# Connor-Guo/torcheval

Hardware: AMD Instinct MI355X
Metric: metric-updates/sec (whole node) MulticlassAccuracy bs=8192 at 1/2/4/8 MI355X (higher is better)
Workload: dtype fp32; 1 GPU; model=MulticlassAccuracy, global_batch=8192, num_classes=1000, batch_per_gpu=8192, average=micro, parallelism=dp1

## Files before the change

csrc/bindings/counts.cpp:

```cpp
#include <ATen/ATen.h>
#include <torch/csrc/utils/pybind.h>
#include <torch/library.h>

#include "tea_kernels.h"
#include "tea_torch.h"

namespace {

using namespace tea_torch;

void cls_counts(const Tensor& input, const Tensor& target, int64_t k, int64_t num_classes,
                const optional<Tensor>& micro_correct, const optional<Tensor>& micro_total,
                const optional<Tensor>& cls_correct, const optional<Tensor>& cls_label,
                const optional<Tensor>& cls_pred, const optional<Tensor>& confusion,
                const optional<Tensor>& err, int64_t max_blocks,
                const optional<Tensor>& micro_incorrect, const optional<Tensor>& micro_total2,
                const optional<Tensor>& cls_fp) {
  check_gpu(input, "input");
  check_gpu(target, "target");
  TORCH_CHECK(target.dim() == 1, "cls_counts: target must be 1-D");
  TORCH_CHECK(input.dim() == 1 || input.dim() == 2, "cls_counts: input must be 1-D or 2-D");
  TORCH_CHECK(input.size(0) == target.size(0), "cls_counts: first dims differ");
  TORCH_CHECK(target.is_contiguous(), "cls_counts: target must be contiguous");
  DeviceGuard guard(input.device());
  tea::ClsCountsArgs a;
  Tensor in = input;
  if (input.dim() == 2) {
    if (in.stride(1) != 1) in = in.contiguous();
    a.c = in.size(1);
    a.row_stride = in.stride(0);
    TORCH_CHECK(a.c < (int64_t(1) << 31), "cls_counts: too many classes");
    TORCH_CHECK(k >= 1 && k <= a.c || a.c == 0, "cls_counts: k out of range");
    if (num_classes <= 0) num_classes = a.c;
    TORCH_CHECK(num_classes == a.c, "cls_counts: num_classes must match input.size(1)");
  } else {
    if (!in.is_contiguous()) in = in.contiguous();
    TORCH_CHECK(k == 1, "cls_counts: k > 1 needs 2-D scores");
  }
  const int64_t C = num_classes;
  a.input = in.data_ptr();
  a.in_dt = dt_of(in);
  a.n = in.size(0);
  a.target = target.data_ptr();
  a.tg_dt = dt_of(target);
  a.k = static_cast<int>(k);
  a.num_classes = C;
  a.micro_correct = f32_out(micro_correct, input, 1, "micro_correct");
  a.micro_total = f32_out(micro_total, input, 1, "micro_total");
  a.cls_correct = f32_out(cls_correct, input, C, "cls_correct");
  a.cls_label = f32_out(cls_label, input, C, "cls_label");
  a.cls_pred = f32_out(cls_pred, input, C, "cls_pred");
  a.confusion = f32_out(confusion, input, C * C, "confusion");
  a.micro_incorrect = f32_out(micro_incorrect, input, 1, "micro_incorrect");
  a.micro_total2 = f32_out(micro_total2, input, 1, "micro_total2");
  a.cls_fp = f32_out(cls_fp, input, C, "cls_fp");
  TORCH_CHECK(!(k > 1 && (a.cls_pred || a.confusion || a.cls_fp)),
              "cls_counts: predictions are undefined for k > 1");
  TORCH_CHECK((a.cls_correct || a.cls_label || a.cls_pred || a.confusion || a.cls_fp) == false ||
                  C > 0,
              "cls_counts: num_classes required for histograms");
  if ((a.err = err_ptr(err, input, "cls_counts")) != nullptr) {
    if (err->numel() >= 3) a.err_max = a.err + 1;
    a.check_target = 1;
  }
  a.max_blocks = static_cast<int>(max_blocks);
  const hipStream_t stream = stream_for(input);
  if (a.micro_correct || a.micro_incorrect) a.fold_ws = fold_workspace(input, stream);
  const int rc = tea::launch_cls_counts(a, stream);
  TORCH_CHECK(rc != -1, "cls_counts: unsupported input dtype ", input.scalar_type());
  check_launch(rc, "cls_counts");
}

bool micro_accuracy_update(const Tensor& input, const Tensor& target, const Tensor& correct,
                           const Tensor& total, int64_t num_classes, const optional<Tensor>& pend) {
  if (!input.is_cuda() || input.dim() != 2 || target.dim() != 1) return false;
  const int64_t n = input.size(0), c = input.size(1);
  if (target.size(0) != n || c <= 0 || c >= (int64_t(1) << 31) || input.stride(1) != 1) return false;
  if (num_classes > 0 && c != num_classes) return false;
  const auto st = input.scalar_type();
  if (st != at::kFloat && st != at::kBFloat16 && st != at::kHalf) return false;
  switch (target.scalar_type()) {
    case at::kLong: case at::kInt: case at::kShort: case at::kChar: case at::kByte: case at::kBool:
      break;
    default: return false;
  }
  if (!target.is_contiguous()) return false;
  const auto dev = input.device();
  if (target.device() != dev || correct.device() != dev || total.device() != dev) return false;
  if (correct.scalar_type() != at::kFloat || total.scalar_type() != at::kFloat ||
      correct.numel() != 1 || total.numel() != 1)
    return false;
  DeviceGuard guard(dev);
  tea::ClsCountsArgs a;
  a.input = input.data_ptr();
  a.in_dt = dt_of(input);
  a.n = n;
  a.c = c;
  a.row_stride = input.stride(0);
  a.target = target.data_ptr();
  a.tg_dt = dt_of(target);
  a.k = 1;
  a.num_classes = c;
  a.micro_correct = correct.data_ptr<float>();
  a.micro_total = total.data_ptr<float>();
  const hipStream_t stream = stream_for(input);
  if (pend.has_value()) {
    if (pend->scalar_type() != at::kLong || pend->numel() < tea::kPendCells * tea::kPendStride ||
        pend->device() != dev || !pend->is_contiguous())
      return false;
    a.pend = reinterpret_cast<unsigned long long*>(pend->data_ptr<int64_t>());
  } else {
    a.fold_ws = fold_workspace(input, stream);
  }
  check_launch(tea::launch_cls_counts(a, stream), "micro_accuracy_update");
  return true;
}

void micro_accuracy_finish(const Tensor& pend, const Tensor& correct, const Tensor& total,
                           const optional<Tensor>& out) {
  check_gpu(pend, "pend");
  TORCH_CHECK(pend.scalar_type() == at::kLong && pend.is_contiguous() &&
                  pend.numel() >= tea::kPendCells * tea::kPendStride,
              "micro_accuracy_finish: pend must be int64 [>= 512]");
  TORCH_CHECK(correct.scalar_type() == at::kFloat && total.scalar_type() == at::kFloat && correct.numel() == 1 &&
                  total.numel() == 1 && correct.device() == pend.device() && total.device() == pend.device(),
              "micro_accuracy_finish: float32 scalar states on the pending cells' device");
  float* o = nullptr;
  if (out.has_value()) {
    TORCH_CHECK(out->scalar_type() == at::kFloat && out->numel() == 1 && out->device() == pend.device(),
                "micro_accuracy_finish: out must be a float32 scalar");
    o = out->data_ptr<float>();
  }
  DeviceGuard guard(pend.device());
  check_launch(tea::launch_micro_finish(reinterpret_cast<unsigned long long*>(pend.data_ptr<int64_t>()),
                                        correct.data_ptr<float>(), total.data_ptr<float>(), o, stream_for(pend)),
               "micro_accuracy_finish");
}

Tensor rank_scores(const Tensor& input, const Tensor& target, int64_t mode, int64_t k,
                   const optional<Tensor>& err) {
  check_gpu(input, "input");
  check_gpu(target, "target");
  TORCH_CHECK(input.dim() == 2 && target.dim() == 1 && input.size(0) == target.size(0),
              "rank_scores: input [n, c] and target [n] expected");
  TORCH_CHECK(mode == 0 || mode == 1, "rank_scores: mode must be 0 (hit) or 1 (reciprocal)");
  TORCH_CHECK(input.size(1) < (int64_t(1) << 31), "rank_scores: too many columns");
  DeviceGuard guard(input.device());
  Tensor in = input.stride(1) == 1 ? input : input.contiguous();
  Tensor tg = target.contiguous();
  tea::RankArgs a;
  a.input = in.data_ptr();
  a.in_dt = dt_of(in);
  a.n = in.size(0);
  a.c = in.size(1);
  a.row_stride = in.stride(0);
  a.target = tg.data_ptr();
  a.tg_dt = dt_of(tg);
  a.mode = static_cast<int>(mode);
  a.k = static_cast<int>(k);
  Tensor out = at::empty({a.n}, input.options().dtype(at::kFloat));
  a.out = out.data_ptr<float>();
  a.err = err_ptr(err, input, "rank_scores");
  const int rc = tea::launch_rank_scores(a, stream_for(input));
  TORCH_CHECK(rc != -1, "rank_scores: unsupported input dtype ", input.scalar_type());
  check_launch(rc, "rank_scores");
  return out;
}

void binary_counts(const Tensor& input, const Tensor& target, const optional<Tensor>& weight,
                   double threshold, const optional<Tensor>& tp, const optional<Tensor>& fp,
                   const optional<Tensor>& tn, const optional<Tensor>& fn,
                   const optional<Tensor>& total, int64_t strict, int64_t max_blocks,
                   const optional<Tensor>& tp2, const optional<Tensor>& fp2,
                   const optional<Tensor>& tn2, const optional<Tensor>& fn2) {
  check_gpu(input, "input");
  check_gpu(target, "target");
  TORCH_CHECK(input.numel() == target.numel(), "binary_counts: size mismatch");
  DeviceGuard guard(input.device());
  Tensor in = input.contiguous();
  Tensor tg = target.contiguous();
  Tensor w;
  tea::BinaryCountsArgs a;
  if (weight.has_value()) {
    w = weight->contiguous();
    TORCH_CHECK(w.numel() == in.numel(), "binary_counts: weight size mismatch");
    a.weight = w.data_ptr();
    a.w_dt = dt_of(w);
  }
  a.input = in.data_ptr();
  a.in_dt = dt_of(in);
  a.target = tg.data_ptr();
  a.tg_dt = dt_of(tg);
  a.n = in.numel();
  a.threshold = threshold_as(in, threshold);
  a.threshold64 = threshold;
  a.strict_binary = static_cast<int>(strict);
  a.out[0] = f32_out(tp, input, 1, "tp");
  a.out[1] = f32_out(fp, input, 1, "fp");
  a.out[2] = f32_out(tn, input, 1, "tn");
  a.out[3] = f32_out(fn, input, 1, "fn");
  a.total = f32_out(total, input, 1, "total");
  a.out2[0] = f32_out(tp2, input, 1, "tp2");
  a.out2[1] = f32_out(fp2, input, 1, "fp2");
  a.out2[2] = f32_out(tn2, input, 1, "tn2");
  a.out2[3] = f32_out(fn2, input, 1, "fn2");
  a.max_blocks = static_cast<int>(max_blocks);
// ... 134 lines not shown
  check_launch(rc, "sample_binned_auroc");
}

void binned_finalize(const Tensor& tp, const Tensor& fp, const optional<Tensor>& fn,
                     const optional<Tensor>& out_auroc, const optional<Tensor>& out_auprc,
                     const optional<Tensor>& out_prec, const optional<Tensor>& out_rec) {
  check_gpu(tp, "tp");
  TORCH_CHECK(tp.dim() == 2 && tp.scalar_type() == at::kFloat && fp.sizes() == tp.sizes() &&
                  fp.strides() == tp.strides() && fp.scalar_type() == at::kFloat,
              "binned_finalize: tp/fp must be float32 [T, rows] with equal strides");
  DeviceGuard guard(tp.device());
  tea::BinnedFinalizeArgs a;
  a.tp = tp.data_ptr<float>();
  a.fp = fp.data_ptr<float>();
  a.k_stride = tp.stride(0);
  a.r_stride = tp.stride(1);
  a.T = static_cast<int>(tp.size(0));
  a.rows = tp.size(1);
  if (out_auprc.has_value()) {
    TORCH_CHECK(fn.has_value() && fn->sizes() == tp.sizes() && fn->strides() == tp.strides() &&
                    fn->scalar_type() == at::kFloat, "binned_finalize: AUPRC needs fn like tp");
    TORCH_CHECK(out_auprc->scalar_type() == at::kFloat && out_auprc->is_contiguous() &&
                    out_auprc->numel() == a.rows, "binned_finalize: out_auprc float32 [rows]");
    a.fn = fn->data_ptr<float>();
    a.out_auprc = out_auprc->data_ptr<float>();
  }
  if (out_auroc.has_value()) {
    TORCH_CHECK(out_auroc->scalar_type() == at::kDouble && out_auroc->is_contiguous() &&
                    out_auroc->numel() == a.rows, "binned_finalize: out_auroc float64 [rows]");
    a.out_auroc = out_auroc->data_ptr<double>();
  }
  if (out_prec.has_value() || out_rec.has_value()) {
    TORCH_CHECK(out_prec.has_value() && out_rec.has_value() && fn.has_value() &&
                    fn->sizes() == tp.sizes() && fn->strides() == tp.strides() &&
                    fn->scalar_type() == at::kFloat,
                "binned_finalize: a curve needs fn like tp and both out_prec / out_rec");
    for (const Tensor* o : {&*out_prec, &*out_rec})
      TORCH_CHECK(o->scalar_type() == at::kFloat && o->is_contiguous() &&
                      o->numel() == a.rows * (a.T + 1) && o->device() == tp.device(),
                  "binned_finalize: curve outputs must be contiguous float32 [rows, T + 1]");
    a.fn = fn->data_ptr<float>();
    a.out_prec = out_prec->data_ptr<float>();
    a.out_rec = out_rec->data_ptr<float>();
  }
  check_launch(tea::launch_binned_finalize(a, stream_for(tp)), "binned_finalize");
}

void op_cls_counts(const Tensor& input, const Tensor& target, int64_t k, int64_t num_classes,
                   const optional<Tensor>& micro_correct, const optional<Tensor>& micro_total,
                   const optional<Tensor>& cls_correct, const optional<Tensor>& cls_label,
                   const optional<Tensor>& cls_pred, const optional<Tensor>& confusion,
                   const optional<Tensor>& err) {
  cls_counts(input, target, k, num_classes, micro_correct, micro_total, cls_correct, cls_label, cls_pred,
             confusion, err, 0, c10::nullopt, c10::nullopt, c10::nullopt);
}
void op_micro_accuracy(const Tensor& input, const Tensor& target, const Tensor& correct, const Tensor& total) {
  TORCH_CHECK(micro_accuracy_update(input, target, correct, total, 0, c10::nullopt),
              "micro_accuracy: unsupported input (needs [N, C] f32/bf16/f16 scores with unit column stride, "
              "[N] integer targets and float32 scalar states on one ROCm device)");
}
void op_binary_counts(const Tensor& input, const Tensor& target, const optional<Tensor>& weight, double threshold,
                      const optional<Tensor>& tp, const optional<Tensor>& fp, const optional<Tensor>& tn,
                      const optional<Tensor>& fn, const optional<Tensor>& total, int64_t strict) {
  binary_counts(input, target, weight, threshold, tp, fp, tn, fn, total, strict, 0, c10::nullopt, c10::nullopt,
                c10::nullopt, c10::nullopt);
}
void op_binned_counts(const Tensor& input, const Tensor& target, const Tensor& thr, int64_t mode, const Tensor& tp,
                      const Tensor& fp, const Tensor& fn, int64_t uniform) {
  binned_counts(input, target, thr, mode, tp, fp, fn, uniform);
}

}

void tea_bind_counts(py::module_& m) {
  m.def("rank_scores", &rank_scores, "K10 rank-of-target scores (hit rate / reciprocal rank)", py::arg("input"),
        py::arg("target"), py::arg("mode"), py::arg("k"), py::arg("err") = py::none());
  m.def("micro_accuracy_update", &micro_accuracy_update,
        "K1 micro accuracy (k=1) accumulated into float32 scalar states; false = not handled", py::arg("input"),
        py::arg("target"), py::arg("correct"), py::arg("total"), py::arg("num_classes") = 0,
        py::arg("pend") = py::none());
  m.def("micro_accuracy_finish", &micro_accuracy_finish,
        "fold the micro kernel's pending cells into correct (and write correct / total to out)", py::arg("pend"),
        py::arg("correct"), py::arg("total"), py::arg("out") = py::none());
  m.def("cls_counts", &cls_counts, "K1 fused classification counts", py::arg("input"), py::arg("target"), py::arg("k"),
        py::arg("num_classes"), py::arg("micro_correct"), py::arg("micro_total"), py::arg("cls_correct"),
        py::arg("cls_label"), py::arg("cls_pred"), py::arg("confusion"), py::arg("err"), py::arg("max_blocks") = 0,
        py::arg("micro_incorrect") = py::none(), py::arg("micro_total2") = py::none(), py::arg("cls_fp") = py::none());
  m.def("binary_counts", &binary_counts, "K1b thresholded binary counts", py::arg("input"), py::arg("target"),
        py::arg("weight"), py::arg("threshold"), py::arg("tp"), py::arg("fp"), py::arg("tn"), py::arg("fn"),
        py::arg("total"), py::arg("strict") = 0, py::arg("max_blocks") = 0, py::arg("tp2") = py::none(),
        py::arg("fp2") = py::none(), py::arg("tn2") = py::none(), py::arg("fn2") = py::none());
  m.def("multilabel_counts", &multilabel_counts, "K2 multilabel accuracy counts", py::arg("input"), py::arg("target"),
        py::arg("threshold"), py::arg("k"), py::arg("criteria"), py::arg("num_correct"),
        py::arg("num_total") = py::none(), py::arg("total") = 0.0);
  m.def("binned_counts", &binned_counts, "K4 binned TP/FP/FN per (threshold, class)", py::arg("input"),
        py::arg("target"), py::arg("thr"), py::arg("mode"), py::arg("tp"), py::arg("fp"), py::arg("fn"),
        py::arg("uniform") = 0);
  m.def("sample_binned_auroc", &sample_binned_auroc,
        "K4b per-sample multiclass binned AUROC (the reference default), labels checked into err", py::arg("input"),
        py::arg("target"), py::arg("thr"), py::arg("out"), py::arg("err"));
  m.def("binned_finalize", &binned_finalize, "binned AUROC / AUPRC / PR-curve points from counts", py::arg("tp"),
        py::arg("fp"), py::arg("fn") = py::none(), py::arg("out_auroc") = py::none(), py::arg("out_auprc") = py::none(),
        py::arg("out_prec") = py::none(), py::arg("out_rec") = py::none());
}

TORCH_LIBRARY_FRAGMENT(torcheval_amd, m) {
  m.def("micro_accuracy(Tensor input, Tensor target, Tensor(a!) correct, Tensor(b!) total) -> ()");
  m.def("cls_counts(Tensor input, Tensor target, int k, int num_classes, Tensor(a!)? micro_correct, "
        "Tensor(b!)? micro_total, Tensor(c!)? cls_correct, Tensor(d!)? cls_label, Tensor(e!)? cls_pred, "
        "Tensor(f!)? confusion, Tensor(g!)? err) -> ()");
  m.def("binary_counts(Tensor input, Tensor target, Tensor? weight, float threshold, Tensor(a!)? tp, "
        "Tensor(b!)? fp, Tensor(c!)? tn, Tensor(d!)? fn, Tensor(e!)? total, int strict) -> ()");
  m.def("multilabel_counts(Tensor input, Tensor target, float threshold, int k, int criteria, "
        "Tensor(a!) num_correct, Tensor(b!)? num_total, float total) -> ()");
  m.def("rank_scores(Tensor input, Tensor target, int score_mode, int k, Tensor(a!)? err) -> Tensor");
  m.def("binned_counts(Tensor input, Tensor target, Tensor thr, int target_mode, Tensor(a!) tp, Tensor(b!) fp, "
        "Tensor(c!) fn, int uniform) -> ()");
  m.def("binned_finalize(Tensor tp, Tensor fp, Tensor? fn, Tensor(a!)? out_auroc, Tensor(b!)? out_auprc, "
        "Tensor(c!)? out_prec, Tensor(d!)? out_rec) -> ()");
}

TORCH_LIBRARY_IMPL(torcheval_amd, CUDA, m) {
  m.impl("micro_accuracy", &op_micro_accuracy);
  m.impl("cls_counts", &op_cls_counts);
  m.impl("binary_counts", &op_binary_counts);
  m.impl("multilabel_counts", &multilabel_counts);
  m.impl("rank_scores", &rank_scores);
  m.impl("binned_counts", &op_binned_counts);
  m.impl("binned_finalize", &binned_finalize);
}

TORCH_LIBRARY_IMPL(torcheval_amd, Meta, m) {
  m.impl("micro_accuracy", &MetaNoop<&op_micro_accuracy>::call);
  m.impl("cls_counts", &MetaNoop<&op_cls_counts>::call);
  m.impl("binary_counts", &MetaNoop<&op_binary_counts>::call);
  m.impl("multilabel_counts", &MetaNoop<&multilabel_counts>::call);
  m.impl("rank_scores", [](const Tensor& input, const Tensor&, int64_t, int64_t, const optional<Tensor>&) {
    return at::empty({input.size(0)}, input.options().dtype(at::kFloat));
  });
  m.impl("binned_counts", &MetaNoop<&op_binned_counts>::call);
  m.impl("binned_finalize", &MetaNoop<&binned_finalize>::call);
}
```

csrc/include/tea_kernels.h:

```cpp
#pragma once

#include <hip/hip_runtime_api.h>
#include <stdint.h>

#include "tea_types.h"

namespace tea {

struct ClsCountsArgs {
  const void* input = nullptr;
  DType in_dt = DType::f32;
  int64_t n = 0;
  int64_t c = 0;
  int64_t row_stride = 0;
  const void* target = nullptr;
  DType tg_dt = DType::i64;
  int k = 1;
  int64_t num_classes = 0;
  float* micro_correct = nullptr;
  float* micro_incorrect = nullptr;
  float* micro_total = nullptr;
  float* micro_total2 = nullptr;
  float* cls_correct = nullptr;
  float* cls_label = nullptr;
  float* cls_pred = nullptr;
  float* cls_fp = nullptr;
  float* confusion = nullptr;
  int* err = nullptr;
  int* err_max = nullptr;
  int check_target = 0;
  unsigned long long* fold_ws = nullptr;
  unsigned long long* pend = nullptr;
  int max_blocks = 0;
};
int launch_cls_counts(const ClsCountsArgs& a, hipStream_t stream);
constexpr int kPendCells = 64;
constexpr int kPendStride = 8;
int launch_micro_finish(unsigned long long* pend, float* correct, const float* total, float* out, hipStream_t stream);

struct BinaryCountsArgs {
  const void* input = nullptr;
  DType in_dt = DType::f32;
  const void* target = nullptr;
  DType tg_dt = DType::f32;
  const void* weight = nullptr;
  DType w_dt = DType::f32;
  int64_t n = 0;
  float threshold = 0.5f;
  double threshold64 = 0.5;
  int strict_binary = 0;
  float* out[4] = {nullptr, nullptr, nullptr, nullptr};
  float* out2[4] = {nullptr, nullptr, nullptr, nullptr};
  float* total = nullptr;
  int max_blocks = 0;
};
int launch_binary_counts(const BinaryCountsArgs& a, hipStream_t stream);

struct RankArgs {
  const void* input = nullptr;
  DType in_dt = DType::f32;
  int64_t n = 0;
  int64_t c = 0;
  int64_t row_stride = 0;
  const void* target = nullptr;
  DType tg_dt = DType::i64;
  int mode = 0;
  int k = 0;
  float* out = nullptr;
  int* err = nullptr;
};
int launch_rank_scores(const RankArgs& a, hipStream_t stream);

}

namespace tea {

struct AucScanArgs {
  int payload_kind = 0;
  const void* sorted = nullptr;
  DType key_dt = DType::f32;
  int64_t key_stride = 0;
  const int64_t* order = nullptr;
  const int32_t* order32 = nullptr;
  int64_t order_stride = 0;
  const void* target = nullptr;
  DType tg_dt = DType::f32;
  int64_t target_stride = 0;
  const void* weight = nullptr;
  DType w_dt = DType::f32;
  int64_t weight_stride = 0;
  int class_mode = 0;
  int64_t rows = 0;
  int64_t n = 0;
  double* out_auroc = nullptr;
  double* out_auprc = nullptr;
  const uint32_t* sort_fault = nullptr;
  const double* init = nullptr;
  double* out_raw = nullptr;
  void* ab = nullptr;
  void* tsum = nullptr;
  void* tstart = nullptr;
  void* tarea = nullptr;
  void* totals = nullptr;
  int32_t* tcnt = nullptr;
  int32_t* cstart = nullptr;
  int64_t* sizes = nullptr;
  const int64_t* row_off = nullptr;
  float* out_prec = nullptr;
  float* out_rec = nullptr;
  void* out_thr = nullptr;
  float min_precision = 0.f;
  float* s_rec = nullptr;
  void* s_thr = nullptr;
  int32_t* gstar = nullptr;
  int32_t* glo = nullptr;
  float* out_max_recall = nullptr;
  void* out_best_thr = nullptr;
};
int64_t auc_scan_workspace_bytes(int64_t rows, int64_t n);
int launch_auc_scan(AucScanArgs a, void* workspace, hipStream_t stream);
// ... 418 lines not shown
```

csrc/kernels/classification.hip:

```cpp
#include <algorithm>
#include <cstdlib>

#include "tea_common.h"
#include "tea_fold.h"
#include "tea_kernels.h"

namespace tea {

namespace {

constexpr int kBlock = 256;
constexpr int kWavesPerBlock = kBlock / kWave;
constexpr int kChunkLoads = 4;
constexpr int kNarrowMaxC = 32;

__device__ __forceinline__ float fmaximum(float a, float b) {
  return __builtin_elementwise_maximum(a, b);
}

template <int KIND>
__device__ __forceinline__ float h16(uint16_t b) {
  return KIND == 1 ? bf16_to_f32(b) : f16_to_f32(b);
}

// ... 243 lines not shown
#pragma unroll
          for (int e = 0; e < VEC; ++e) v[u][e] = nx[u][e];
        if (base + CHUNK < C) load_chunk<KIND, VEC, UNAL>(rp, base + CHUNK, C, lane, nx);
        finish_chunk<VEC, UNAL>(v, base, C, lane);
        float m = v[0][0];
#pragma unroll
        for (int u = 0; u < kChunkLoads; ++u)
#pragma unroll
          for (int e = 0; e < VEC; ++e) m = fmaximum(m, v[u][e]);
        int idx = 0x7fffffff;
#pragma unroll
        for (int u = kChunkLoads - 1; u >= 0; --u)
#pragma unroll
          for (int e = VEC - 1; e >= 0; --e)
            idx = (v[u][e] == m) ? (base + u * STEP + lane * VEC + e) : idx;
        saw_nan |= (m != m);
        if (m > bv || bi == 0x7fffffff) {
          bv = m;
          bi = idx;
        }
      }
      float wm = bv;
#pragma unroll
      for (int o = 32; o > 0; o >>= 1) wm = fmaximum(wm, __shfl_xor(wm, o, kWave));
      int widx = (bv == wm) ? bi : 0x7fffffff;
#pragma unroll
      for (int o = 32; o > 0; o >>= 1) widx = min(widx, __shfl_xor(widx, o, kWave));
      if (__builtin_expect(__any(saw_nan), 0)) widx = row_argmax_exact<KIND>(rp, C, lane);
      pred = widx;
      correct = pred == t;
    } else {
      t = load_target(a.target, a.tg_dt, row);
      const bool t_ok = t >= 0 && t < C;
      const float xt = t_ok ? load_one<KIND>(rp, t) : __builtin_nanf("");
      int cnt = 0;
      float nx[kChunkLoads][VEC];
      load_chunk<KIND, VEC, UNAL>(rp, 0, C, lane, nx);
      for (int base = 0; base < C; base += CHUNK) {
        float v[kChunkLoads][VEC];
#pragma unroll
        for (int u = 0; u < kChunkLoads; ++u)
#pragma unroll
          for (int e = 0; e < VEC; ++e) v[u][e] = nx[u][e];
        if (base + CHUNK < C) load_chunk<KIND, VEC, UNAL>(rp, base + CHUNK, C, lane, nx);
        finish_chunk<VEC, UNAL>(v, base, C, lane);
#pragma unroll
        for (int u = 0; u < kChunkLoads; ++u)
#pragma unroll
          for (int e = 0; e < VEC; ++e) cnt += v[u][e] > xt;
      }
      cnt = wave_sum(cnt);
      correct = t_ok && cnt < a.k;
    }
    if (lane == 0) {
      correct_acc += correct;
      rows_acc += 1;
      row_hist(h, a.num_classes, t, pred, correct, a.err, a.check_target, a.err_max);
    }
  }
  block_micro(a, correct_acc, rows_acc);
}


template <int CTRL>
__device__ __forceinline__ float dpp_f32(float x) {
  return __int_as_float(__builtin_amdgcn_update_dpp(0, __float_as_int(x), CTRL, 0xf, 0xf, false));
}

__device__ __forceinline__ float wave_max_dpp(float x) {
  x = fmaximum(x, dpp_f32<0xB1>(x));
  x = fmaximum(x, dpp_f32<0x4E>(x));
  x = fmaximum(x, dpp_f32<0x141>(x));
  x = fmaximum(x, dpp_f32<0x140>(x));
  const float r0 = __int_as_float(__builtin_amdgcn_readlane(__float_as_int(x), 0));
  const float r1 = __int_as_float(__builtin_amdgcn_readlane(__float_as_int(x), 16));
  const float r2 = __int_as_float(__builtin_amdgcn_readlane(__float_as_int(x), 32));
  const float r3 = __int_as_float(__builtin_amdgcn_readlane(__float_as_int(x), 48));
  return fmaximum(fmaximum(r0, r1), fmaximum(r2, r3));
}

template <int NV>
struct RowVals;
template <>
struct RowVals<16> {
  typedef float type __attribute__((ext_vector_type(16)));
};
template <>
struct RowVals<32> {
  typedef float type __attribute__((ext_vector_type(32)));
};

template <int KIND, typename TGT, bool UNAL = false>
__device__ __forceinline__ void micro_rows(const void* __restrict__ input, const TGT* __restrict__ target, int64_t n,
                                           int C, int64_t row_stride, uint32_t& correct_acc, uint32_t& rows_acc) {
  constexpr int VEC = KIND == 0 ? 4 : 8;
  constexpr int NV = kChunkLoads * VEC;
  constexpr int STEP = kWave * VEC;
  constexpr int ELSIZE = KIND == 0 ? 4 : 2;
  typedef typename RowVals<NV>::type vec_t;
  const int lane = lane_id();
  const int64_t nwaves = static_cast<int64_t>(gridDim.x) * kWavesPerBlock;
  for (int64_t row = static_cast<int64_t>(blockIdx.x) * kWavesPerBlock + wave_id(); row < n; row += nwaves) {
    const char* rp = static_cast<const char*>(input) + row * row_stride * ELSIZE;
    float f[kChunkLoads][VEC];
#pragma unroll
    for (int u = 0; u < kChunkLoads; ++u) load_row_vec<KIND, VEC, UNAL>(rp, u * STEP + lane * VEC, C, f[u]);
    const int64_t t = target[row];
    if constexpr (UNAL) unal_fix_tail<kChunkLoads>(f, 0, C, lane);
    vec_t v;
#pragma unroll
    for (int u = 0; u < kChunkLoads; ++u)
#pragma unroll
      for (int e = 0; e < VEC; ++e) v[u * VEC + e] = f[u][e];
    float m = fmaximum(v[0], v[1]);
#pragma unroll
    for (int e = 2; e < NV; ++e) m = fmaximum(m, v[e]);
    const float wm = wave_max_dpp(m);
    bool correct = false;
    if (__builtin_expect(wm != wm, 0)) {
      correct = row_argmax_exact<KIND>(rp, C, lane) == t;
    } else if (t >= 0 && t < C) {
      const int tu = static_cast<int>(t);
      const float sel = v[(tu / STEP) * VEC + (tu % VEC)];
      const float xt = __int_as_float(__builtin_amdgcn_readlane(__float_as_int(sel), (tu % STEP) / VEC));
      if (xt == wm) {
        int cnt = 0;
#pragma unroll
        for (int u = 0; u < kChunkLoads; ++u) {
          const int valid = min(max((C - u * STEP + VEC - 1) / VEC, 0), kWave);
          const uint64_t lanes = valid >= kWave ? ~0ull : ((1ull << valid) - 1);
#pragma unroll
          for (int e = 0; e < VEC; ++e) cnt += __builtin_popcountll(__ballot(v[u * VEC + e] == wm) & lanes);
        }
        correct = cnt == 1 || row_argmax_exact<KIND>(rp, C, lane) == t;
      }
    }
    if (lane == 0) {
      correct_acc += correct;
      rows_acc += 1;
    }
  }
}

template <int KIND, typename TGT, bool UNAL>
__global__ __launch_bounds__(kBlock) void cls_micro_kernel(ClsCountsArgs a) {
  uint32_t correct_acc = 0, rows_acc = 0;
  micro_rows<KIND, TGT, UNAL>(a.input, static_cast<const TGT*>(a.target), a.n, static_cast<int>(a.c), a.row_stride,
                        correct_acc, rows_acc);
  block_micro(a, correct_acc, rows_acc);
}

struct MicroPendArgs {
  const void* input;
  const void* target;
  unsigned long long* pend;
  float* total;
  int64_t n;
  int64_t row_stride;
  int32_t c;
  int32_t pad;
};

template <int KIND, typename TGT, bool UNAL>
__device__ __forceinline__ bool micro_row(const MicroPendArgs& a, const char* __restrict__ rp, int64_t t, int lane) {
  constexpr int VEC = KIND == 0 ? 4 : 8;
  constexpr int NV = kChunkLoads * VEC;
  constexpr int STEP = kWave * VEC;
  typedef typename RowVals<NV>::type vec_t;
  const int C = a.c;
  float f[kChunkLoads][VEC];
#pragma unroll
  for (int u = 0; u < kChunkLoads; ++u) load_row_vec<KIND, VEC, UNAL>(rp, u * STEP + lane * VEC, C, f[u]);
  if constexpr (UNAL) unal_fix_tail<kChunkLoads>(f, 0, C, lane);
  vec_t v;
#pragma unroll
  for (int u = 0; u < kChunkLoads; ++u)
#pragma unroll
    for (int e = 0; e < VEC; ++e) v[u * VEC + e] = f[u][e];
  float m = fmaximum(v[0], v[1]);
#pragma unroll
  for (int e = 2; e < NV; ++e) m = fmaximum(m, v[e]);
  if (__builtin_expect(__ballot(m != m) != 0, 0)) return row_argmax_exact<KIND>(rp, C, lane) == t;
  if (!(t >= 0 && t < C)) return false;
  const int tu = static_cast<int>(t);
  const float sel = v[(tu / STEP) * VEC + (tu % VEC)];
  const float xt = __int_as_float(__builtin_amdgcn_readlane(__float_as_int(sel), (tu % STEP) / VEC));
  if (__ballot(m > xt) != 0) return false;
  bool tie = false;
#pragma unroll
  for (int u = 0; u < kChunkLoads; ++u)
#pragma unroll
    for (int e = 0; e < VEC; ++e) tie |= (v[u * VEC + e] == xt) & (u * STEP + lane * VEC + e < tu);
  return __ballot(tie) == 0;
}

template <int KIND, typename TGT, int WPB, bool UNAL>
__global__ __launch_bounds__(WPB * kWave) void cls_micro_pend_kernel(MicroPendArgs a) {
  constexpr int ELSIZE = KIND == 0 ? 4 : 2;
  const int lane = lane_id();
  const int64_t nwaves = static_cast<int64_t>(gridDim.x) * WPB;
  const int64_t row0 = static_cast<int64_t>(blockIdx.x) * WPB + wave_id();
  const int64_t r0 = row0 < a.n ? row0 : a.n - 1;
  const bool c0 = micro_row<KIND, TGT, UNAL>(a, static_cast<const char*>(a.input) + r0 * a.row_stride * ELSIZE,
                                       static_cast<const TGT*>(a.target)[r0], lane);
  uint32_t correct_acc = (row0 < a.n && c0) ? 1u : 0u;
  for (int64_t row = row0 + nwaves; row < a.n; row += nwaves) {
    const char* rp = static_cast<const char*>(a.input) + row * a.row_stride * ELSIZE;
    correct_acc += micro_row<KIND, TGT, UNAL>(a, rp, static_cast<const TGT*>(a.target)[row], lane);
  }
  if (lane == 0 && correct_acc)
    atomicAdd(a.pend + ((blockIdx.x * WPB + wave_id()) % kPendCells) * kPendStride,
              static_cast<unsigned long long>(correct_acc));
  if (blockIdx.x == 0 && threadIdx.x == 0 && a.total) atomicAdd(a.total, static_cast<float>(a.n));
}

__global__ __launch_bounds__(kWave) void micro_finish_kernel(unsigned long long* pend, float* correct,
                                                             const float* total, float* out) {
  unsigned long long* cell = pend + threadIdx.x * kPendStride;
  const unsigned long long s = wave_sum(*cell);
  *cell = 0ull;
  if (threadIdx.x == 0) {
    const float c = correct[0] + static_cast<float>(s);
    correct[0] = c;
    if (out) out[0] = c / total[0];
  }
}

template <int KIND, int VEC, bool TOPK, bool PRED = true, bool UNAL = false>
__global__ __launch_bounds__(kBlock) void cls_wide_kernel(ClsCountsArgs a) {
  cls_wide_body<KIND, VEC, TOPK, PRED, UNAL>(a);
}

template <int KIND, bool TOPK>
__global__ __launch_bounds__(kBlock) void cls_narrow_kernel(ClsCountsArgs a) {
  constexpr int ELSIZE = KIND == 0 ? 4 : 2;
  __shared__ float s_correct[kNarrowMaxC], s_label[kNarrowMaxC], s_pred[kNarrowMaxC];
  __shared__ float s_fp[kNarrowMaxC];
  __shared__ float s_conf[kNarrowMaxC * kNarrowMaxC];
  const int C = static_cast<int>(a.c);
  for (int i = threadIdx.x; i < C * C; i += kBlock) s_conf[i] = 0.f;
  if (threadIdx.x < kNarrowMaxC) {
    s_correct[threadIdx.x] = 0.f;
    s_label[threadIdx.x] = 0.f;
    s_pred[threadIdx.x] = 0.f;
    s_fp[threadIdx.x] = 0.f;
  }
  __syncthreads();
  const Hist lh{a.cls_correct ? s_correct : nullptr, a.cls_label ? s_label : nullptr,
                a.cls_pred ? s_pred : nullptr, a.cls_fp ? s_fp : nullptr,
                a.confusion ? s_conf : nullptr};
  uint32_t correct_acc = 0, rows_acc = 0;
  const int64_t stride = static_cast<int64_t>(gridDim.x) * kBlock;
  for (int64_t row = static_cast<int64_t>(blockIdx.x) * kBlock + threadIdx.x; row < a.n;
       row += stride) {
    const void* rp = static_cast<const char*>(a.input) + row * a.row_stride * ELSIZE;
    const int64_t t = load_target(a.target, a.tg_dt, row);
    bool correct;
    int64_t pred = -1;
    if constexpr (!TOPK) {
      float bv = -__builtin_huge_valf();
      int bi = 0x7fffffff;
      for (int c = 0; c < C; ++c) {
        const float v = load_one<KIND>(rp, c);
        if (argmax_better(v, c, bv, bi)) {
          bv = v;
          bi = c;
        }
      }
      pred = bi;
      correct = pred == t;
    } else {
      const bool t_ok = t >= 0 && t < C;
      const float xt = t_ok ? load_one<KIND>(rp, t) : __builtin_nanf("");
      int cnt = 0;
      for (int c = 0; c < C; ++c) cnt += load_one<KIND>(rp, c) > xt;
      correct = t_ok && cnt < a.k;
    }
    correct_acc += correct;
    rows_acc += 1;
    row_hist(lh, C, t, pred, correct, a.err, a.check_target, a.err_max);
  }
  __syncthreads();
  for (int i = threadIdx.x; i < C; i += kBlock) {
    if (a.cls_correct && s_correct[i] != 0.f) atomicAdd(a.cls_correct + i, s_correct[i]);
    if (a.cls_label && s_label[i] != 0.f) atomicAdd(a.cls_label + i, s_label[i]);
    if (a.cls_pred && s_pred[i] != 0.f) atomicAdd(a.cls_pred + i, s_pred[i]);
    if (a.cls_fp && s_fp[i] != 0.f) atomicAdd(a.cls_fp + i, s_fp[i]);
  }
  if (a.confusion)
    for (int i = threadIdx.x; i < C * C; i += kBlock)
      if (s_conf[i] != 0.f) atomicAdd(a.confusion + i, s_conf[i]);
  block_micro(a, correct_acc, rows_acc);
}

__global__ __launch_bounds__(kBlock) void cls_labels_kernel(ClsCountsArgs a) {
// ... 156 lines not shown
```

torcheval_amd/metrics/classification/accuracy.py:

```python

from typing import Iterable, Optional, TypeVar

import torch

from torcheval_amd.metrics.functional.classification.accuracy import (
    _CPU_FAST_MAX,
    _accuracy_compute,
    _accuracy_param_check,
    _accuracy_update_input_check,
    _binary_accuracy_update,
    _binary_accuracy_update_input_check,
    _multiclass_accuracy_update_aten,
    _multilabel_accuracy_param_check,
    _multilabel_accuracy_update,
    _multilabel_accuracy_update_input_check,
    _topk_multilabel_accuracy_param_check,
    _topk_multilabel_accuracy_update,
    _topk_multilabel_accuracy_update_input_check,
    _cpu_binary_ok,
    _cpu_fast_ok,
)
from torcheval_amd.metrics.metric import Metric, inference_update
import torcheval_amd.ops as _ops
from torcheval_amd.ops import compiling, native, native_loaded, use_native
# ... 58 lines not shown
        self.k = k
        self._err: Optional[torch.Tensor] = None
        self._pend: Optional[torch.Tensor] = None
        self._pend_id = 0
        self._pend_dirty = False
        shape = () if average == "micro" else (num_classes or 0,)
        self._add_state("num_correct", torch.zeros(shape, device=self.device), merge="sum")
        self._add_state("num_total", torch.zeros(shape, device=self.device), merge="sum")
        self._refresh_fast_path()

    @property
    def _err_words(self) -> int:
        return 0 if self.average == "micro" and self.k == 1 else 1

    def _refresh_fast_path(self) -> None:
        self._fast = (
            _FAST_MICRO is not None
            and not _ops.DISABLE_HIP
            and self.average == "micro"
            and self.k == 1
            and type(self) is MulticlassAccuracy
            and self._device.type == "cuda"
        )
        self._fast_nc = self.num_classes or 0

    def to(self: TAccuracy, device, *args, **kwargs) -> TAccuracy:
        super().to(device, *args, **kwargs)
        self._pend = None
        self._refresh_fast_path()
        return self

    def _get_num_correct(self) -> torch.Tensor:
        d = self.__dict__
        if d.get("_pend_dirty"):
            self._fold_pending()
        return d["_nc"]

    def _set_num_correct(self, value: torch.Tensor) -> None:
        d = self.__dict__
        if d.get("_pend_dirty"):
            d["_pend"].zero_()
            d["_pend_dirty"] = False
        d["_nc"] = value

    num_correct = property(_get_num_correct, _set_num_correct)

    def _fold_pending(self, out: Optional[torch.Tensor] = None) -> None:
        d = self.__dict__
        native().micro_accuracy_finish(d["_pend"], d["_nc"], d["num_total"], out)
        d["_pend_dirty"] = False

    def _mark_updated(self, captured=None) -> None:
        if self.__dict__.get("_pend") is not None:
            self.__dict__["_pend_dirty"] = True

    def _raw_state(self, name: str) -> torch.Tensor:
        return self.__dict__["_nc"] if name == "num_correct" else getattr(self, name)

    def __getstate__(self):
        d = self.__dict__
        if d.get("_pend_dirty"):
            self._fold_pending()
        state = dict(d)
        state["_pend"] = None
        state["_pend_dirty"] = False
        return state

    def __setstate__(self, state) -> None:
        self.__dict__.update(state)

    def reset(self: TAccuracy) -> TAccuracy:
        d = self.__dict__
        if d.get("_pend_dirty"):
            d["_pend"].zero_()
            d["_pend_dirty"] = False
        return super().reset()

    def update(self: TAccuracy, input: torch.Tensor, target: torch.Tensor) -> TAccuracy:
        if self._fast:
            if not compiling():
                d = self.__dict__
                pend = d["_pend"]
                if pend is None or d["_pend_id"] != id(self):
                    pend = d["_pend"] = torch.zeros(512, dtype=torch.int64, device=self._device)
                    d["_pend_id"] = id(self)
                if _FAST_MICRO(input, target, d["_nc"], d["num_total"], self._fast_nc, pend):
                    d["_pend_dirty"] = True
                    return self
            elif _micro_op_ok(input, target, self.num_correct, self._fast_nc):
                torch.ops.torcheval_amd.micro_accuracy(input, target, self.num_correct, self.num_total)
                return self
        dev = self._device
        if input.device != dev:
            input = input.to(dev)
        if target.device != dev:
            target = target.to(dev)
        _accuracy_update_input_check(input, target, self.num_classes, self.k)
        if (
            self.average == "micro"
            and not input.is_cuda
            and input.numel() <= _CPU_FAST_MAX
            and self.num_correct.dtype == torch.float32
            and _cpu_fast_ok(input, target, self.k, None)
        ):
            native().cpu_micro_accuracy_update(input, target, self.k, self.num_correct, self.num_total)
            return self
        if native_cls(input, target, self.num_correct, self.num_total,
                      num_classes=None if self.average == "micro" else self.num_classes):
            if self.average == "micro":
                if self.k > 1 and self._err is None:
                    self._err = torch.zeros(1, dtype=torch.int32, device=dev)
                cls_counts(
                    input,
                    target,
                    k=self.k,
                    num_classes=input.shape[1] if input.ndim == 2 else 0,
                    micro_correct=self.num_correct,
                    micro_total=self.num_total,
                    err=self._err,
                )
            else:
                if self._err is None:
                    self._err = torch.zeros(1, dtype=torch.int32, device=dev)
                cls_counts(
                    input,
                    target,
                    k=self.k,
                    num_classes=self.num_classes,
                    cls_correct=self.num_correct,
                    cls_label=self.num_total,
                    err=self._err,
                )
            return self
        with torch.inference_mode():
            num_correct, num_total = _multiclass_accuracy_update_aten(
                input, target, self.average, self.num_classes, self.k
            )
            self.num_correct += num_correct
            self.num_total += num_total
        return self

    def _check_device_errors(self) -> None:
        _raise_on_device_error(self._err)

    def compute(self: TAccuracy) -> torch.Tensor:
        d = self.__dict__
        if d.get("_pend_dirty"):
            out = torch.empty((), dtype=torch.float32, device=d["num_total"].device)
            self._fold_pending(out)
        elif self.average == "micro" or self.average is None or self.average == "none":
            out = self.num_correct / self.num_total
        else:
            with torch.inference_mode():
                out = _accuracy_compute(self.num_correct, self.num_total, self.average)
        self._check_device_errors()
        return out

    @torch.inference_mode()
    def merge_state(self: TAccuracy, metrics: Iterable[TAccuracy]) -> TAccuracy:
        for metric in metrics:
            self.num_correct += metric.num_correct.to(self.device)
            self.num_total += metric.num_total.to(self.device)
        return self


class BinaryAccuracy(MulticlassAccuracy):

# ... 124 lines not shown
```

Measured before the change: 164,100 updates/s.

## Add adaptive early-exit mode to micro accuracy kernel using a running hint

Measured after the change: 239,300 updates/s (median of 6 runs). 1.46x the previous value.

```diff
diff --git a/csrc/bindings/counts.cpp b/csrc/bindings/counts.cpp
--- a/csrc/bindings/counts.cpp
+++ b/csrc/bindings/counts.cpp
@@ -1,6 +1,8 @@
 #include <ATen/ATen.h>
 #include <torch/csrc/utils/pybind.h>
 #include <torch/library.h>
+
+#include <tuple>
 
 #include "tea_kernels.h"
 #include "tea_torch.h"
@@ -105,7 +107,7 @@
   a.micro_total = total.data_ptr<float>();
   const hipStream_t stream = stream_for(input);
   if (pend.has_value()) {
-    if (pend->scalar_type() != at::kLong || pend->numel() < tea::kPendCells * tea::kPendStride ||
+    if (pend->scalar_type() != at::kLong || pend->numel() < tea::kPendWords ||
         pend->device() != dev || !pend->is_contiguous())
       return false;
     a.pend = reinterpret_cast<unsigned long long*>(pend->data_ptr<int64_t>());
@@ -120,8 +122,8 @@
                            const optional<Tensor>& out) {
   check_gpu(pend, "pend");
   TORCH_CHECK(pend.scalar_type() == at::kLong && pend.is_contiguous() &&
-                  pend.numel() >= tea::kPendCells * tea::kPendStride,
-              "micro_accuracy_finish: pend must be int64 [>= 512]");
+                  pend.numel() >= tea::kPendWords,
+              "micro_accuracy_finish: pend must be int64 [>= ", tea::kPendWords, "]");
   TORCH_CHECK(correct.scalar_type() == at::kFloat && total.scalar_type() == at::kFloat && correct.numel() == 1 &&
                   total.numel() == 1 && correct.device() == pend.device() && total.device() == pend.device(),
               "micro_accuracy_finish: float32 scalar states on the pending cells' device");
@@ -422,6 +424,18 @@
   m.def("micro_accuracy_finish", &micro_accuracy_finish,
         "fold the micro kernel's pending cells into correct (and write correct / total to out)", py::arg("pend"),
         py::arg("correct"), py::arg("total"), py::arg("out") = py::none());
+  m.def("_micro_hint_slot", [] { return tea::kPendHintSlot; },
+        "word index of the micro kernel's mode hint {rows_seen, correct_seen} in the pending buffer");
+  m.def("_micro_first_phase_loads", [] { return tea::kMicroFirstPhaseLoads; },
+        "wave-loads (of 4 per row) the micro kernel issues before the hint and the target are known");
+  m.def("_micro_hint_rule",
+        [](unsigned long long rows_seen, unsigned long long correct_seen) {
+          return std::make_tuple(tea::micro_hint_early(rows_seen, correct_seen),
+                                 rows_seen - tea::micro_hint_decay(rows_seen, rows_seen),
+                                 correct_seen - tea::micro_hint_decay(rows_seen, correct_seen));
+        },
+        "the hint rule on the host: (early mode?, rows_seen after decay, correct_seen after decay)",
+        py::arg("rows_seen"), py::arg("correct_seen"));
   m.def("cls_counts", &cls_counts, "K1 fused classification counts", py::arg("input"), py::arg("target"), py::arg("k"),
         py::arg("num_classes"), py::arg("micro_correct"), py::arg("micro_total"), py::arg("cls_correct"),
         py::arg("cls_label"), py::arg("cls_pred"), py::arg("confusion"), py::arg("err"), py::arg("max_blocks") = 0,
diff --git a/csrc/include/tea_kernels.h b/csrc/include/tea_kernels.h
--- a/csrc/include/tea_kernels.h
+++ b/csrc/include/tea_kernels.h
@@ -36,6 +36,17 @@
 int launch_cls_counts(const ClsCountsArgs& a, hipStream_t stream);
 constexpr int kPendCells = 64;
 constexpr int kPendStride = 8;
+constexpr int kPendHintSlot = kPendCells * kPendStride;
+constexpr int kPendWords = kPendHintSlot + kPendStride;
+constexpr int kMicroFirstPhaseLoads = 1;
+constexpr unsigned long long kMicroHintMinRows = 64;
+constexpr unsigned long long kMicroHintDecayRows = 4096;
+constexpr bool micro_hint_early(unsigned long long rows_seen, unsigned long long correct_seen) {
+  return rows_seen >= kMicroHintMinRows && 4 * correct_seen < rows_seen;
+}
+constexpr unsigned long long micro_hint_decay(unsigned long long rows_seen, unsigned long long word) {
+  return rows_seen >= kMicroHintDecayRows ? word - word / 2 : 0ull;
+}
 int launch_micro_finish(unsigned long long* pend, float* correct, const float* total, float* out, hipStream_t stream);
 
 struct BinaryCountsArgs {
diff --git a/csrc/kernels/classification.hip b/csrc/kernels/classification.hip
--- a/csrc/kernels/classification.hip
+++ b/csrc/kernels/classification.hip
@@ -349,6 +349,14 @@
 template <int NV>
 struct RowVals;
 template <>
+struct RowVals<4> {
+  typedef float type __attribute__((ext_vector_type(4)));
+};
+template <>
+struct RowVals<8> {
+  typedef float type __attribute__((ext_vector_type(8)));
+};
+template <>
 struct RowVals<16> {
   typedef float type __attribute__((ext_vector_type(16)));
 };
@@ -428,22 +436,74 @@
   int32_t pad;
 };
 
+template <int NVALS, int VEC, typename V>
+__device__ __forceinline__ bool lane_tie_before(const V& v, float xt, int tu, int lane) {
+  int k = 1 << 20;
+#pragma unroll
+  for (int e = NVALS - 1; e >= 0; --e) k = (v[e] == xt) ? e : k;
+  return (k / VEC) * (kWave * VEC) + lane * VEC + (k % VEC) < tu;
+}
+
+template <int KIND, bool UNAL>
+__device__ __forceinline__ void micro_row_head(const char* __restrict__ rp, int C, int lane,
+                                               float (&f)[kMicroFirstPhaseLoads][KIND == 0 ? 4 : 8]) {
+  constexpr int VEC = KIND == 0 ? 4 : 8;
+#pragma unroll
+  for (int u = 0; u < kMicroFirstPhaseLoads; ++u)
+    load_row_vec<KIND, VEC, UNAL>(rp, u * kWave * VEC + lane * VEC, C, f[u]);
+}
+
 template <int KIND, typename TGT, bool UNAL>
-__device__ __forceinline__ bool micro_row(const MicroPendArgs& a, const char* __restrict__ rp, int64_t t, int lane) {
+__device__ __forceinline__ bool micro_row(const MicroPendArgs& a, const char* __restrict__ rp,
+                                          float (&f)[kMicroFirstPhaseLoads][KIND == 0 ? 4 : 8], int64_t t, bool early,
+                                          int lane) {
   constexpr int VEC = KIND == 0 ? 4 : 8;
   constexpr int NV = kChunkLoads * VEC;
   constexpr int STEP = kWave * VEC;
+  constexpr int P = kMicroFirstPhaseLoads, Q = kChunkLoads - P;
+  static_assert(P >= 1 && Q >= 1, "both phases hold at least one wave-load");
   typedef typename RowVals<NV>::type vec_t;
+  typedef typename RowVals<P * VEC>::type head_t;
   const int C = a.c;
-  float f[kChunkLoads][VEC];
-#pragma unroll
-  for (int u = 0; u < kChunkLoads; ++u) load_row_vec<KIND, VEC, UNAL>(rp, u * STEP + lane * VEC, C, f[u]);
-  if constexpr (UNAL) unal_fix_tail<kChunkLoads>(f, 0, C, lane);
+  float g[Q][VEC];
+  if (early) {
+    if (!(t >= 0 && t < C)) return false;
+    const int tu = static_cast<int>(t);
+    const bool t_loaded = tu < P * STEP;
+    float xt = 0.f;
+    if (!t_loaded) xt = load_one<KIND>(rp, tu);
+    if constexpr (UNAL) unal_fix_tail<P>(f, 0, C, lane);
+    head_t h;
+#pragma unroll
+    for (int u = 0; u < P; ++u)
+#pragma unroll
+      for (int e = 0; e < VEC; ++e) h[u * VEC + e] = f[u][e];
+    if (t_loaded) {
+      const float sel = h[(tu / STEP) * VEC + (tu % VEC)];
+      xt = __int_as_float(__builtin_amdgcn_readlane(__float_as_int(sel), (tu % STEP) / VEC));
+    }
+    float hm = h[P * VEC - 1];
+#pragma unroll
+    for (int e = P * VEC - 2; e >= 0; --e) hm = fmaximum(hm, h[e]);
+    if (__ballot(hm > xt) != 0) return false;
+    if (__ballot(lane_tie_before<P * VEC, VEC>(h, xt, tu, lane)) != 0) return false;
+#pragma unroll
+    for (int u = 0; u < Q; ++u) load_row_vec<KIND, VEC, UNAL>(rp, (P + u) * STEP + lane * VEC, C, g[u]);
+  } else {
+#pragma unroll
+    for (int u = 0; u < Q; ++u) load_row_vec<KIND, VEC, UNAL>(rp, (P + u) * STEP + lane * VEC, C, g[u]);
+    if constexpr (UNAL) unal_fix_tail<P>(f, 0, C, lane);
+  }
+  if constexpr (UNAL) unal_fix_tail<Q>(g, P * STEP, C, lane);
   vec_t v;
 #pragma unroll
-  for (int u = 0; u < kChunkLoads; ++u)
+  for (int u = 0; u < P; ++u)
 #pragma unroll
     for (int e = 0; e < VEC; ++e) v[u * VEC + e] = f[u][e];
+#pragma unroll
+  for (int u = 0; u < Q; ++u)
+#pragma unroll
+    for (int e = 0; e < VEC; ++e) v[(P + u) * VEC + e] = g[u][e];
   float m = fmaximum(v[0], v[1]);
 #pragma unroll
   for (int e = 2; e < NV; ++e) m = fmaximum(m, v[e]);
@@ -453,12 +513,7 @@
   const float sel = v[(tu / STEP) * VEC + (tu % VEC)];
   const float xt = __int_as_float(__builtin_amdgcn_readlane(__float_as_int(sel), (tu % STEP) / VEC));
   if (__ballot(m > xt) != 0) return false;
-  bool tie = false;
-#pragma unroll
-  for (int u = 0; u < kChunkLoads; ++u)
-#pragma unroll
-    for (int e = 0; e < VEC; ++e) tie |= (v[u * VEC + e] == xt) & (u * STEP + lane * VEC + e < tu);
-  return __ballot(tie) == 0;
+  return __ballot(lane_tie_before<NV, VEC>(v, xt, tu, lane)) == 0;
 }
 
 template <int KIND, typename TGT, int WPB, bool UNAL>
@@ -468,16 +523,38 @@
   const int64_t nwaves = static_cast<int64_t>(gridDim.x) * WPB;
   const int64_t row0 = static_cast<int64_t>(blockIdx.x) * WPB + wave_id();
   const int64_t r0 = row0 < a.n ? row0 : a.n - 1;
-  const bool c0 = micro_row<KIND, TGT, UNAL>(a, static_cast<const char*>(a.input) + r0 * a.row_stride * ELSIZE,
-                                       static_cast<const TGT*>(a.target)[r0], lane);
+  const char* rp0 = static_cast<const char*>(a.input) + r0 * a.row_stride * ELSIZE;
+  const int64_t t0 = static_cast<const TGT*>(a.target)[r0];
+  const unsigned long long seen = a.pend[kPendHintSlot], seen_correct = a.pend[kPendHintSlot + 1];
+  __builtin_amdgcn_sched_barrier(0);
+  float f[kMicroFirstPhaseLoads][KIND == 0 ? 4 : 8];
+  micro_row_head<KIND, UNAL>(rp0, a.c, lane, f);
+  __builtin_amdgcn_sched_barrier(0);
+  const bool early = micro_hint_early(seen, seen_correct);
+  const bool c0 = micro_row<KIND, TGT, UNAL>(a, rp0, f, t0, early, lane);
   uint32_t correct_acc = (row0 < a.n && c0) ? 1u : 0u;
+  uint32_t rows_acc = row0 < a.n ? 1u : 0u;
   for (int64_t row = row0 + nwaves; row < a.n; row += nwaves) {
     const char* rp = static_cast<const char*>(a.input) + row * a.row_stride * ELSIZE;
-    correct_acc += micro_row<KIND, TGT, UNAL>(a, rp, static_cast<const TGT*>(a.target)[row], lane);
+    micro_row_head<KIND, UNAL>(rp, a.c, lane, f);
+    correct_acc += micro_row<KIND, TGT, UNAL>(a, rp, f, static_cast<const TGT*>(a.target)[row], early, lane);
+    rows_acc += 1;
   }
   if (lane == 0 && correct_acc)
     atomicAdd(a.pend + ((blockIdx.x * WPB + wave_id()) % kPendCells) * kPendStride,
               static_cast<unsigned long long>(correct_acc));
+  if (blockIdx.x == 0 && lane == 0) {
+    unsigned long long* hint = a.pend + kPendHintSlot;
+    unsigned long long dr = 0ull, dc = 0ull;
+    if (wave_id() == 0) {
+      const unsigned long long r = __hip_atomic_load(hint, __ATOMIC_RELAXED, __HIP_MEMORY_SCOPE_AGENT);
+      const unsigned long long c = __hip_atomic_load(hint + 1, __ATOMIC_RELAXED, __HIP_MEMORY_SCOPE_AGENT);
+      dr = micro_hint_decay(r, r);
+      dc = micro_hint_decay(r, c);
+    }
+    if (rows_acc != dr) atomicAdd(hint, static_cast<unsigned long long>(rows_acc) - dr);
+    if (correct_acc != dc) atomicAdd(hint + 1, static_cast<unsigned long long>(correct_acc) - dc);
+  }
   if (blockIdx.x == 0 && threadIdx.x == 0 && a.total) atomicAdd(a.total, static_cast<float>(a.n));
 }
 
diff --git a/torcheval_amd/metrics/classification/accuracy.py b/torcheval_amd/metrics/classification/accuracy.py
--- a/torcheval_amd/metrics/classification/accuracy.py
+++ b/torcheval_amd/metrics/classification/accuracy.py
@@ -164,7 +164,7 @@
                 d = self.__dict__
                 pend = d["_pend"]
                 if pend is None or d["_pend_id"] != id(self):
-                    pend = d["_pend"] = torch.zeros(512, dtype=torch.int64, device=self._device)
+                    pend = d["_pend"] = torch.zeros(520, dtype=torch.int64, device=self._device)
                     d["_pend_id"] = id(self)
                 if _FAST_MICRO(input, target, d["_nc"], d["num_total"], self._fast_nc, pend):
                     d["_pend_dirty"] = True
```
